# LBANN/DGraph

Measured on AMD Instinct MI355X. Metric: edges_per_s, higher is better.
Workload: dtype fp32

## Files before the change

### csrc/bindings_f32.cpp

```cpp
#include <algorithm>
#include <mutex>
#include <vector>
#include <set>
#include <tuple>
#include <ATen/ATen.h>
#include <c10/core/DeviceGuard.h>
#include <c10/hip/HIPStream.h>
#include <torch/library.h>

#include "check.h"
#include "kernels/kernels.h"

namespace dgraph {
namespace {

hipStream_t stream_of(const at::Tensor& t) {
  return c10::hip::getCurrentHIPStream(t.device().index()).stream();
}

void same_dev(const at::Tensor& t, const at::Tensor& ref, const char* name) {
  TORCH_CHECK(t.is_cuda() && t.device() == ref.device(), "dgraph_amd: ", name,
              " must be a GPU tensor on ", ref.device());
}

// ... 39 lines not shown
              "col must be contiguous int32/int64");
  TORCH_CHECK(x.size(1) == out.size(1), "x/out feature mismatch");
  const at::Tensor* ri = opt(row_ids);
  const at::Tensor* re = opt(rowend);
  const int64_t csr_rows = re ? re->numel() : rowptr.numel() - 1;
  if (re) {
    same_dev(*re, x, "rowend");
    TORCH_CHECK(re->scalar_type() == at::kLong && re->is_contiguous() &&
                    rowptr.numel() >= re->numel(),
                "rowend must be contiguous int64 with at most rowptr's entries");
  }
  const int64_t nrows = ri ? ri->numel() : csr_rows;
  const int64_t* rid = idx64(row_ids, x, nrows, "row_ids");
  const int64_t* rmap = idx64(row_map, x, nrows, "row_map");
  if (!rmap) TORCH_CHECK(out.size(0) >= nrows, "out has fewer rows than the CSR rows");
  auto f32opt = [&](const c10::optional<at::Tensor>& t, const char* name) -> const float* {
    const at::Tensor* p = opt(t);
    if (!p) return nullptr;
    same_dev(*p, x, name);
    TORCH_CHECK(p->scalar_type() == at::kFloat && p->is_contiguous(), name,
                " must be contiguous float32");
    return p->data_ptr<float>();
  };
  SpmmF32Args a;
  a.rowptr = rowptr.data_ptr<int64_t>();
  a.rowend = re ? re->data_ptr<int64_t>() : nullptr;
  a.col = col.data_ptr();
  a.it = col.scalar_type() == at::kInt ? IType::I32 : IType::I64;
  a.ew = f32opt(ew, "edge_weight");
  if (a.ew) TORCH_CHECK(ew->numel() == col.numel(), "edge_weight must be [E]");
  a.col_scale = f32opt(cs, "col_scale");
  a.row_scale = f32opt(rs, "row_scale");
  if (const at::Tensor* p = opt(cmap)) {
    same_dev(*p, x, "col_map");
    TORCH_CHECK(p->scalar_type() == at::kInt && p->is_contiguous(),
                "col_map must be contiguous int32");
    a.col_map = p->data_ptr<int32_t>();
  }
  TORCH_CHECK(spmm_f32_rowgroup_ok(static_cast<int>(x.size(1)), x.stride(0), out.stride(0),
                                   x.data_ptr(), out.data_ptr()),
              "spmm_f32_ex: F % 4 == 0 and 16-B aligned rows/strides required");
  if (const at::Tensor* p = opt(x2)) {
    f32_rows(*p, "x2");
    same_dev(*p, x, "x2");
    TORCH_CHECK(p->size(1) == x.size(1) && p->stride(0) % 4 == 0 &&
                    reinterpret_cast<uintptr_t>(p->data_ptr()) % 16 == 0,
                "x2 must be 16-B aligned, as wide as x, row stride % 4 == 0");
    TORCH_CHECK(nsplit >= 0 && nsplit <= x.size(0) && nsplit < (int64_t(1) << 32),
                "nsplit must be in [0, rows of x]");
    TORCH_CHECK(!a.ew && !a.col_scale,
                "x2 (two sources) is not combined with edge weights / col_scale");
    a.x2 = p->data_ptr<float>();
    a.ldx2 = p->stride(0);
    a.nsplit = nsplit;
  }
  if (const at::Tensor* gt = opt(gate)) {
    f32_rows(*gt, "gate");
    same_dev(*gt, x, "gate");
    TORCH_CHECK(gt->size(1) >= x.size(1) && gt->stride(0) % 4 == 0 &&
                    reinterpret_cast<uintptr_t>(gt->data_ptr()) % 16 == 0,
                "gate must be 16-B aligned with row stride % 4 == 0, width >= F");
    if (!rmap) TORCH_CHECK(gt->size(0) >= nrows, "gate has fewer rows than the output");
    a.gate = gt->data_ptr<float>();
    a.ldgate = gt->stride(0);
  }
  if (const at::Tensor* sa = opt(self_add)) {
    f32_rows(*sa, "self_add");
    same_dev(*sa, x, "self_add");
    const at::Tensor* sm = opt(self_map);
    TORCH_CHECK(sm != nullptr, "self_add needs self_map");
    same_dev(*sm, x, "self_map");
    TORCH_CHECK(sm->scalar_type() == at::kInt && sm->is_contiguous(),
                "self_map must be contiguous int32");
    TORCH_CHECK(sa->size(1) >= x.size(1) && sa->stride(0) % 4 == 0 &&
                    reinterpret_cast<uintptr_t>(sa->data_ptr()) % 16 == 0,
                "self_add must be 16-B aligned with row stride % 4 == 0, width >= F");
    const int64_t max_out = rmap ? out.size(0) : nrows;
    TORCH_CHECK(self_row0 >= 0 && self_row0 + max_out <= sm->numel(),
                "self_map too short for self_row0 + output rows");
    if (sa->size(0) > 0) {
      a.self_add = sa->data_ptr<float>();
      a.self_map = sm->data_ptr<int32_t>();
      a.ld_self = sa->stride(0);
      a.self_row0 = self_row0;
    }
  }
  a.row_ids = rid;
  a.row_map = rmap;
  a.x = x.data_ptr<float>();
  a.ldx = x.stride(0);
  a.out = out.data_ptr<float>();
  a.ldo = out.stride(0);
  a.nrows = nrows;
  a.F = static_cast<int>(x.size(1));
  a.beta = static_cast<float>(beta);
  a.cap = cap;
  a.pass_cols = static_cast<int>(pass_cols);
  if (const at::Tensor* kb = opt(keep_bits)) {
    same_dev(*kb, x, "keep_bits");
    TORCH_CHECK(kb->scalar_type() == at::kInt && kb->dim() == 2 && kb->stride(1) == 1,
                "keep_bits must be int32 [rows, words] with unit column stride");
    TORCH_CHECK(kb->size(1) * 32 >= x.size(1), "keep_bits narrower than the columns");
    TORCH_CHECK(kb->size(0) >= (rmap ? out.size(0) : nrows),
                "keep_bits has fewer rows than the output rows");
    a.keep_bits = reinterpret_cast<const uint32_t*>(kb->data_ptr<int32_t>());
    a.ld_bits = kb->stride(0);
  }
  c10::DeviceGuard g(x.device());
  DG_HIP_CHECK(spmm_f32_run(a, stream_of(x)));
}

void gemm_f32_op(const at::Tensor& A1, const at::Tensor& B1, const c10::optional<at::Tensor>& A2,
                 const c10::optional<at::Tensor>& B2, const c10::optional<at::Tensor>& a_rows,
                 const c10::optional<at::Tensor>& bias, const c10::optional<at::Tensor>& cin,
                 double beta, const c10::optional<at::Tensor>& gate,
                 const c10::optional<at::Tensor>& o_rows, bool relu, const at::Tensor& out,
                 const c10::optional<at::Tensor>& row_scale,
                 const c10::optional<at::Tensor>& send_out,
                 const c10::optional<at::Tensor>& send_ptr,
                 const c10::optional<at::Tensor>& send_pos) {
  f32_rows(A1, "A1");
  f32_rows(B1, "B1");
  f32_rows(out, "out");
  same_dev(B1, A1, "B1");
  same_dev(out, A1, "out");
  const at::Tensor* ar = opt(a_rows);
  const int64_t M = ar ? ar->numel() : A1.size(0);
  const int64_t N = B1.size(1), K1 = A1.size(1);
  TORCH_CHECK(B1.size(0) == K1, "gemm_f32: A1/B1 inner dimension mismatch");
  TORCH_CHECK(out.size(1) == N, "gemm_f32: out width != N");
  TORCH_CHECK(A1.size(0) <= INT32_MAX && M <= INT32_MAX, "gemm_f32: more than 2^31 rows");
  const int64_t* arp = idx64(a_rows, A1, M, "a_rows");
  const int64_t* orp = idx64(o_rows, A1, M, "o_rows");
  if (!orp) TORCH_CHECK(out.size(0) >= M, "gemm_f32: out has fewer than M rows");
  const at::Tensor *a2 = opt(A2), *b2 = opt(B2);
  TORCH_CHECK((a2 == nullptr) == (b2 == nullptr), "gemm_f32: A2 and B2 go together");
  int64_t K2 = 0;
  if (a2) {
    f32_rows(*a2, "A2");
    f32_rows(*b2, "B2");
    same_dev(*a2, A1, "A2");
    same_dev(*b2, A1, "B2");
    K2 = a2->size(1);
    TORCH_CHECK(b2->size(0) == K2 && b2->size(1) == N, "gemm_f32: A2/B2 shape mismatch");
    TORCH_CHECK(a2->size(0) >= M, "gemm_f32: A2 has fewer than M rows");
// ... 191 lines not shown
  DG_HIP_CHECK(apply_keep_bits(g.data_ptr<float>(), g.stride(0),
                               reinterpret_cast<const uint32_t*>(bits.data_ptr<int32_t>()),
                               n, F, stream_of(g), rp));
}

void xent_rows_op(const at::Tensor& z, const at::Tensor& rows, const at::Tensor& y,
                  double scale, const at::Tensor& dz, const at::Tensor& row_loss, int64_t C) {
  f32_rows(z, "z");
  f32_rows(dz, "dz");
  same_dev(rows, z, "rows");
  same_dev(y, z, "y");
  same_dev(dz, z, "dz");
  same_dev(row_loss, z, "row_loss");
  const int64_t n = rows.numel();
  TORCH_CHECK(rows.scalar_type() == at::kLong && rows.is_contiguous() &&
                  y.scalar_type() == at::kLong && y.is_contiguous() && y.numel() == n,
              "rows / y must be contiguous int64 of equal length");
  TORCH_CHECK(C > 0 && C <= 256 && C <= z.size(1) && dz.size(1) >= C && dz.size(1) <= 256 &&
                  dz.size(0) >= n,
              "xent_rows: C <= 256, z and dz at least C wide, dz >= n rows");
  TORCH_CHECK(row_loss.scalar_type() == at::kFloat && row_loss.is_contiguous() &&
                  row_loss.numel() >= n,
              "row_loss must be contiguous float32 with >= n entries");
  c10::DeviceGuard g(z.device());
  DG_HIP_CHECK(xent_rows(z.data_ptr<float>(), z.stride(0), static_cast<int>(C),
                         rows.data_ptr<int64_t>(), y.data_ptr<int64_t>(), n,
                         static_cast<float>(scale), dz.data_ptr<float>(), dz.stride(0),
                         static_cast<int>(dz.size(1)), row_loss.data_ptr<float>(), stream_of(z)));
}

void argmax_hits_op(const at::Tensor& z, const at::Tensor& rows, const at::Tensor& y,
                    const at::Tensor& hit, int64_t C) {
  f32_rows(z, "z");
  same_dev(rows, z, "rows");
  same_dev(y, z, "y");
  same_dev(hit, z, "hit");
  const int64_t n = rows.numel();
  TORCH_CHECK(rows.scalar_type() == at::kLong && rows.is_contiguous() &&
                  y.scalar_type() == at::kLong && y.is_contiguous() && y.numel() == n,
              "rows / y must be contiguous int64 of equal length");
  TORCH_CHECK(hit.scalar_type() == at::kByte && hit.is_contiguous() && hit.numel() >= n,
              "hit must be contiguous uint8 with >= n entries");
  TORCH_CHECK(C > 0 && C <= 256 && C <= z.size(1), "argmax_hits: 0 < C <= 256, C <= width");
  c10::DeviceGuard g(z.device());
  DG_HIP_CHECK(argmax_hits(z.data_ptr<float>(), z.stride(0), static_cast<int>(C),
                           rows.data_ptr<int64_t>(), y.data_ptr<int64_t>(), n,
                           hit.data_ptr<uint8_t>(), stream_of(z)));
}

void set_spmm_f32_config_op(int64_t rowgroup, int64_t pass_cols) {
  set_spmm_f32_config(static_cast<int>(rowgroup), static_cast<int>(pass_cols));
}

void set_f32_sched_op(int64_t spmm_grid, int64_t dynamic, int64_t spmm_xcd) {
  if (spmm_grid >= 0) set_spmm_f32_grid(static_cast<int>(spmm_grid));
  if (spmm_xcd >= 0) set_spmm_f32_xcd(static_cast<int>(spmm_xcd));
  if (dynamic >= 0) set_f32_dynamic(dynamic != 0);
}

void f32_init_op() { DG_HIP_CHECK(work_counters_init()); }

}
}

TORCH_LIBRARY_FRAGMENT(dgraph_amd, m) {
  m.def("set_f32_sched(int spmm_grid=-1, int dynamic=-1, int spmm_xcd=-1) -> ()", &dgraph::set_f32_sched_op);
  m.def("f32_init() -> ()", &dgraph::f32_init_op);
  m.def("set_spmm_f32_config(int rowgroup, int pass_cols=-1) -> ()",
        &dgraph::set_spmm_f32_config_op);
  m.def("spmm_f32_ex(Tensor rowptr, Tensor col, Tensor? edge_weight, Tensor? col_scale, "
        "Tensor? row_scale, Tensor? col_map, Tensor? row_ids, Tensor x, Tensor(a!) out, "
        "float beta=0., int cap=0, Tensor? row_map=None, Tensor? gate=None, "
        "Tensor? self_add=None, Tensor? self_map=None, int self_row0=0, Tensor? rowend=None, "
        "Tensor? x2=None, int nsplit=0, int pass_cols=0, Tensor? keep_bits=None) -> ()");
  m.def("gemm_f32(Tensor A1, Tensor B1, Tensor? A2, Tensor? B2, Tensor? a_rows, Tensor? bias, "
        "Tensor? cin, float beta, Tensor? gate, Tensor? o_rows, bool relu, Tensor(a!) out, "
        "Tensor? row_scale=None, Tensor(b!)? send_out=None, Tensor? send_ptr=None, "
        "Tensor? send_pos=None) -> ()");
  m.def("wgrad_f32(Tensor A1, Tensor? A2, Tensor? a1_rows, Tensor G, Tensor(a!) partials, "
        "int blocks, int fresh_from, Tensor(b!)? col_partials=None) -> ()");
  m.def("wgrad_f32_reduce(Tensor partials, Tensor(a!) out) -> ()");
  m.def("row_keep_bits(Tensor h, Tensor? rows, Tensor(a!) bits) -> ()");
  m.def("apply_keep_bits(Tensor(a!) g, Tensor bits, Tensor? rows=None) -> ()");
  m.def("xent_rows(Tensor z, Tensor rows, Tensor y, float scale, Tensor(a!) dz, "
        "Tensor(b!) row_loss, int C) -> ()");
  m.def("argmax_hits(Tensor z, Tensor rows, Tensor y, Tensor(a!) hit, int C) -> ()");
}

TORCH_LIBRARY_IMPL(dgraph_amd, CUDA, m) {
  m.impl("spmm_f32_ex", &dgraph::spmm_f32_ex_op);
  m.impl("gemm_f32", &dgraph::gemm_f32_op);
  m.impl("wgrad_f32", &dgraph::wgrad_f32_op);
  m.impl("wgrad_f32_reduce", &dgraph::wgrad_f32_reduce_op);
  m.impl("row_keep_bits", &dgraph::row_keep_bits_op);
  m.impl("apply_keep_bits", &dgraph::apply_keep_bits_op);
  m.impl("xent_rows", &dgraph::xent_rows_op);
  m.impl("argmax_hits", &dgraph::argmax_hits_op);
}
```

### csrc/kernels/kernels.h

```cpp
#pragma once
#include <hip/hip_runtime.h>
#include <stdint.h>

#include <initializer_list>

namespace dgraph {

enum class DType : int { F32 = 0, BF16 = 1 };
enum class IType : int { I32 = 0, I64 = 1 };

void set_spmm_config(int variant, int xcd, int pass_cols);

hipError_t spmm_csr(DType dt, IType it, const int64_t* rowptr, const void* col,
                    const float* ew, int heads, int head_dim, const float* col_scale,
                    const float* row_scale, const void* x, int64_t ldx, void* out,
                    int64_t ldo, int64_t nrows, int F, float beta, hipStream_t stream,
                    int64_t cap = 0, const int64_t* row_map = nullptr);

bool spmm_f32_rowgroup_ok(int F, int64_t ldx, int64_t ldo, const void* x, const void* out);
hipError_t spmm_f32_rowgroup(IType it, const int64_t* rowptr, const void* col,
                             const float* ew, const float* col_scale, const float* row_scale,
                             const int32_t* col_map, const int64_t* row_ids, const float* x,
                             int64_t ldx, float* out, int64_t ldo, int64_t nrows, int F,
                             float beta, int64_t cap, const int64_t* row_map,
                             hipStream_t st, const float* gate = nullptr, int64_t ldgate = 0,
                             const float* self_add = nullptr, int64_t ld_self = 0,
                             const int32_t* self_map = nullptr, int64_t self_row0 = 0);
struct SpmmF32Args {
  const int64_t* rowptr = nullptr;
  const int64_t* rowend = nullptr;
  const void* col = nullptr;
  IType it = IType::I32;
  const float* ew = nullptr;
  const float* col_scale = nullptr;
  const float* row_scale = nullptr;
  const int32_t* col_map = nullptr;
  const int64_t* row_ids = nullptr;
  const int64_t* row_map = nullptr;
  const float* x = nullptr;
  int64_t ldx = 0;
  const float* x2 = nullptr;
  int64_t ldx2 = 0;
  int64_t nsplit = 0;
  float* out = nullptr;
  int64_t ldo = 0;
  int64_t nrows = 0;
  int F = 0;
  float beta = 0.f;
  int64_t cap = 0;
  const float* gate = nullptr;
  int64_t ldgate = 0;
  const float* self_add = nullptr;
  int64_t ld_self = 0;
  const int32_t* self_map = nullptr;
  int64_t self_row0 = 0;
  int pass_cols = 0;
  int xcd_remap = 0;
  const uint32_t* keep_bits = nullptr;
  int64_t ld_bits = 0;
  int bits_col0 = 0;
};
hipError_t spmm_f32_run(const SpmmF32Args& a, hipStream_t st);
void set_spmm_f32_pass_cols(int cols);
void set_spmm_f32_config(int rowgroup, int pass_cols);
void set_spmm_f32_grid(int blocks);
void set_spmm_f32_xcd(int on);

hipError_t spmm_hub_partials(DType dt, IType it, const int64_t* seg_beg,
                             const int64_t* seg_end, const void* col, const float* ew,
                             const float* col_scale, const void* x, int64_t ldx,
                             float* partials, int64_t nseg, int F, hipStream_t stream);
hipError_t spmm_hub_reduce(DType dt, const float* partials, const int64_t* hub_seg_ptr,
                           const int64_t* hub_rows, const float* row_scale, void* out,
                           int64_t ldo, int64_t nhub, int F, hipStream_t stream);

hipError_t segment_extreme_fwd(DType dt, IType it, bool minimum, const int64_t* rowptr,
                               const void* col, const void* x, int64_t ldx, void* out,
                               int64_t ldo, int32_t* arg, int64_t lda, int64_t nrows, int F,
                               bool second, const int64_t* row_map, hipStream_t stream);
hipError_t segment_extreme_bwd(DType dt, IType it, const int64_t* t_rowptr, const void* t_col,
                               const int32_t* rel, const void* g, int64_t ldg,
                               const int32_t* arg, int64_t lda, void* out, int64_t ldo,
                               int64_t nrows, int F, bool halo, float beta,
                               hipStream_t stream);

hipError_t segment_pna_fwd(IType it, const int64_t* rowptr, const void* col, const float* x,
                           int64_t ldx, float* mean, int64_t ld_mean, float* sdev,
                           int64_t ld_sdev, float* vmax, int64_t ld_vmax, int32_t* amax,
                           int64_t ld_amax, float* vmin, int64_t ld_vmin, int32_t* amin,
                           int64_t ld_amin, int64_t nrows, int F, float eps, bool second,
                           bool final, const int64_t* prev_rowptr, const int64_t* row_map,
                           hipStream_t stream);
hipError_t segment_pna_bwd(IType it, const int64_t* t_rowptr, const void* t_col,
                           const int32_t* rel, const float* x, int64_t ldx,
                           const float* inv_deg, const float* g_mean, int64_t ld_gmean,
                           const float* g_std, int64_t ld_gstd, const float* mean,
                           int64_t ld_mean, const float* sdev, int64_t ld_sdev,
                           const float* g_max, int64_t ld_gmax, const int32_t* amax,
                           int64_t ld_amax, const float* g_min, int64_t ld_gmin,
                           const int32_t* amin, int64_t ld_amin, float* out, int64_t ldo,
                           int64_t nrows, int F, bool halo, float beta, hipStream_t stream);

int64_t segment_softmax_dt_parts(int64_t nrows);
hipError_t segment_softmax_fwd(IType it, const int64_t* rowptr, const void* col, const float* x,
                               int64_t ldx, const float* t, float* out, int64_t ldo, float* lse,
                               int64_t ldl, int64_t nrows, int F, bool second,
                               const int64_t* row_map, hipStream_t stream);
hipError_t segment_softmax_bwd(IType it, const int64_t* t_rowptr, const void* t_col,
                               const float* x, int64_t ldx, const float* t, const float* g,
                               int64_t ldg, const float* out_fwd, int64_t ldof,
                               const float* lse, int64_t ldl, float* dx, int64_t lddx,
                               float* dt_part, int64_t nrows, int F, hipStream_t stream);

int64_t segment_softmax_edge_dt_parts(int64_t nrows);
hipError_t segment_softmax_edge_fwd(IType it, const int64_t* rowptr, const void* col,
                                    const float* x, int64_t ldx, const float* e, int64_t lde,
                                    const float* t, float* out, int64_t ldo, float* lse,
                                    int64_t ldl, int64_t nrows, int F, bool relu, float eps,
                                    bool second, const int64_t* row_map, hipStream_t stream);
// ... 268 lines not shown
```

### csrc/kernels/spmm_f32.hip

```cpp
#include "../common.h"
#include "kernels.h"

namespace dgraph {
namespace {

typedef float f32x2 __attribute__((ext_vector_type(2)));

template <typename IdxT, int LPR, int WMODE, bool CMAP, bool TWO, bool KB = false,
          bool GS = false>
__global__ __launch_bounds__(256) void spmm_f32_rowgroup_kernel(SpmmF32Args a) {
  constexpr int VEC = 4;
  constexpr int G = kWave / LPR;
  constexpr int U = LPR < 8 ? LPR : 8;
  constexpr bool HAS_EW = (WMODE & 1) != 0;
  constexpr bool HAS_CS = (WMODE & 2) != 0;
  const IdxT* __restrict__ col = static_cast<const IdxT*>(a.col);
  const int64_t* __restrict__ rowptr = a.rowptr;
  const int lane = threadIdx.x & (kWave - 1);
  const int g = lane / LPR;
  const int l = lane % LPR;
  const int wv = threadIdx.x >> 6;
  __shared__ uint8_t inv[CMAP ? 4 * 64 : 1];
  const int64_t nrows = a.nrows;
  const int F = a.F;
  const int64_t ngroups = (nrows + G - 1) / G;
  int64_t blk = blockIdx.x;
  if (a.xcd_remap) {
    const int64_t full = static_cast<int64_t>(gridDim.x) & ~int64_t(7);
    if (blk < full) blk = (blk & 7) * (full >> 3) + (blk >> 3);
  }
  const int64_t q0 = (blk * blockDim.x + threadIdx.x) >> 6;
  const int64_t qstep = (static_cast<int64_t>(gridDim.x) * blockDim.x) >> 6;
  const int f = l * VEC;
  const bool active = f < F;
  const float* xf = a.x + (active ? f : 0);
  const float* x2f = TWO ? a.x2 + (active ? f : 0) : nullptr;
  const uint64_t ldx = static_cast<uint64_t>(a.ldx);
  const uint64_t ldx2 = static_cast<uint64_t>(a.ldx2);
  const uint32_t ns = static_cast<uint32_t>(a.nsplit);
  const int cap = a.cap;
  auto row_ptr = [&](uint32_t c) -> const float* {
    if constexpr (TWO) {
      return c < ns ? xf + static_cast<uint64_t>(c) * ldx
                    : x2f + static_cast<uint64_t>(c - ns) * ldx2;
    } else {
      return xf + static_cast<uint64_t>(c) * ldx;
    }
  };
  for (int64_t q = q0; q < ngroups; q += qstep) {
    const int64_t r = q * G + g;
    const bool has_row = r < nrows;
    const int64_t rr = has_row ? (a.row_ids ? a.row_ids[r] : r) : 0;
    const int64_t s = has_row ? rowptr[rr] : 0;
    const int64_t deg1 = has_row ? (a.rowend ? a.rowend[rr] : rowptr[rr + 1]) - s : 0;
    const int deg = static_cast<int>(deg1 > cap ? cap : deg1);
    int32_t m_top = -1;
    if constexpr (GS) m_top = a.self_map[a.self_row0 + (has_row ? r : 0)];
    int maxdeg = deg;
#pragma unroll
    for (int off = LPR; off < kWave; off <<= 1) {
      const int o = __shfl_xor(maxdeg, off, kWave);
      maxdeg = o > maxdeg ? o : maxdeg;
    }
    f32x2 acc[VEC / 2];
#pragma unroll
    for (int i = 0; i < VEC / 2; ++i) acc[i] = f32x2{0.f, 0.f};
    auto load_c = [&](int k) -> int64_t {
      const IdxT c = col[k < deg ? s + k : 0];
      return k < deg ? static_cast<int64_t>(c) : int64_t(0);
    };
    auto load_w = [&](int64_t& c, int k) -> float {
      float w = k < deg ? 1.f : 0.f;
      if constexpr (CMAP) {
        const int32_t m = a.col_map[c];
        w = m >= 0 ? w : 0.f;
        c = m >= 0 ? m : 0;
      }
      if constexpr (HAS_EW) w *= a.ew[k < deg ? s + k : 0];
      if constexpr (HAS_CS) w *= a.col_scale[c];
      return w;
    };
    int64_t my_c = 0;
    float my_w = 0.f;
    if (maxdeg > 0) {
      my_c = load_c(l);
      my_w = load_w(my_c, l);
    }
    for (int k0 = 0; k0 < maxdeg; k0 += LPR) {
      const int kn = k0 + LPR + l;
// ... 19 lines not shown
#pragma unroll
          for (int u = 0; u < U; ++u) {
            const int j = j0 + u;
            const int src = j < cnt ? static_cast<int>(inv[wv * kWave + g * LPR + j]) : 0;
            c[u] = static_cast<uint32_t>(__shfl(static_cast<int>(my_c), g * LPR + src, kWave));
            const float ww = __shfl(my_w, g * LPR + src, kWave);
            w[u] = j < cnt ? ww : 0.f;
          }
#pragma unroll
          for (int u = 0; u < U; ++u) v[u] = *reinterpret_cast<const uint4*>(row_ptr(c[u]));
#pragma unroll
          for (int u = 0; u < U; ++u) {
            const f32x2 ww{w[u], w[u]};
            const f32x2 t0{__uint_as_float(v[u].x), __uint_as_float(v[u].y)};
            const f32x2 t1{__uint_as_float(v[u].z), __uint_as_float(v[u].w)};
            acc[0] = __builtin_elementwise_fma(t0, ww, acc[0]);
            acc[1] = __builtin_elementwise_fma(t1, ww, acc[1]);
          }
        }
        my_w = load_w(nx_c, kn);
        my_c = nx_c;
        continue;
      }
#pragma unroll
      for (int j0 = 0; j0 < LPR; j0 += U) {
        if (j0 > 0 && k0 + j0 >= maxdeg) break;
        uint4 v[U];
        uint32_t c[U];
        float w[U];
#pragma unroll
        for (int u = 0; u < U; ++u)
          c[u] = static_cast<uint32_t>(
              __shfl(static_cast<int>(my_c), g * LPR + j0 + u, kWave));
        if (j0 == 0) nx_c = load_c(kn);
#pragma unroll
        for (int u = 0; u < U; ++u) v[u] = *reinterpret_cast<const uint4*>(row_ptr(c[u]));
#pragma unroll
        for (int u = 0; u < U; ++u) w[u] = __shfl(my_w, g * LPR + j0 + u, kWave);
#pragma unroll
        for (int u = 0; u < U; ++u) {
          const f32x2 ww{w[u], w[u]};
          const f32x2 t0{__uint_as_float(v[u].x), __uint_as_float(v[u].y)};
          const f32x2 t1{__uint_as_float(v[u].z), __uint_as_float(v[u].w)};
          acc[0] = __builtin_elementwise_fma(t0, ww, acc[0]);
          acc[1] = __builtin_elementwise_fma(t1, ww, acc[1]);
        }
      }
      my_w = load_w(nx_c, kn);
      my_c = nx_c;
    }
    if (has_row && active) {
      const int64_t orow = (!GS && a.row_map) ? a.row_map[r] : r;
      const float rs = a.row_scale ? a.row_scale[orow] : 1.f;
      float* o = a.out + orow * a.ldo + f;
      const float beta = a.beta;
      float4 res;
      if (beta != 0.f) {
        const float4 old = *reinterpret_cast<const float4*>(o);
        res.x = fmaf(acc[0].x, rs, beta * old.x);
        res.y = fmaf(acc[0].y, rs, beta * old.y);
        res.z = fmaf(acc[1].x, rs, beta * old.z);
        res.w = fmaf(acc[1].y, rs, beta * old.w);
      } else {
        res.x = acc[0].x * rs;
        res.y = acc[0].y * rs;
        res.z = acc[1].x * rs;
        res.w = acc[1].y * rs;
      }
      if constexpr (GS) {
        const float4 sv = *reinterpret_cast<const float4*>(
            a.self_add + static_cast<int64_t>(m_top >= 0 ? m_top : 0) * a.ld_self + f);
        const float4 gv = *reinterpret_cast<const float4*>(a.gate + orow * a.ldgate + f);
        res.x = m_top >= 0 ? res.x + sv.x : res.x;
        res.y = m_top >= 0 ? res.y + sv.y : res.y;
        res.z = m_top >= 0 ? res.z + sv.z : res.z;
        res.w = m_top >= 0 ? res.w + sv.w : res.w;
        res.x = gv.x > 0.f ? res.x : 0.f;
        res.y = gv.y > 0.f ? res.y : 0.f;
        res.z = gv.z > 0.f ? res.z : 0.f;
        res.w = gv.w > 0.f ? res.w : 0.f;
      } else if (a.self_add) {
        const int32_t m = a.self_map[a.self_row0 + orow];
        if (m >= 0) {
          const float4 sv = *reinterpret_cast<const float4*>(a.self_add + m * a.ld_self + f);
          res.x += sv.x;
          res.y += sv.y;
          res.z += sv.z;
          res.w += sv.w;
        }
      }
      if (!GS && a.gate) {
        const float4 gv = *reinterpret_cast<const float4*>(a.gate + orow * a.ldgate + f);
        res.x = gv.x > 0.f ? res.x : 0.f;
        res.y = gv.y > 0.f ? res.y : 0.f;
        res.z = gv.z > 0.f ? res.z : 0.f;
        res.w = gv.w > 0.f ? res.w : 0.f;
      }
      if constexpr (KB) {
        const int c = a.bits_col0 + f;
        const uint32_t w = a.keep_bits[orow * a.ld_bits + (c >> 5)] >> (c & 31);
        res.x = (w & 1u) ? res.x : 0.f;
        res.y = (w & 2u) ? res.y : 0.f;
        res.z = (w & 4u) ? res.z : 0.f;
        res.w = (w & 8u) ? res.w : 0.f;
      }
      *reinterpret_cast<float4*>(o) = res;
    }
  }
}

int g_f32_grid_cap = 0;
int g_f32_xcd = 0;

template <typename IdxT>
hipError_t launch_f32_rg(const SpmmF32Args& a, hipStream_t st) {
  const int lanes = (a.F + 3) / 4;
  const int LPR = lanes <= 8 ? 8 : lanes <= 16 ? 16 : lanes <= 32 ? 32 : 64;
  const int64_t G = kWave / LPR;
  const int64_t ngroups = (a.nrows + G - 1) / G;
  int64_t blocks = (ngroups + 3) / 4;
  SpmmF32Args ka = a;
  ka.xcd_remap = g_f32_xcd ? 1 : 0;
  if (g_f32_grid_cap > 0 && blocks > g_f32_grid_cap) {
    blocks = g_f32_grid_cap;
    ka.xcd_remap = 0;
  }
  if (blocks > 0x7fffffff) return hipErrorInvalidValue;
  const int wmode = (a.ew != nullptr ? 1 : 0) | (a.col_scale != nullptr ? 2 : 0);
  const bool cmap = a.col_map != nullptr;
  const bool two = a.x2 != nullptr;
  const bool kb = a.keep_bits != nullptr;
  if (two && wmode != 0) return hipErrorInvalidValue;
  if (kb && (two || cmap || wmode != 0)) return hipErrorInvalidValue;
  if (kb) {
#define DG_F32_KB(LPR_)                                                                      \
    if (LPR == LPR_) {                                                                       \
      hipLaunchKernelGGL((spmm_f32_rowgroup_kernel<IdxT, LPR_, 0, false, false, true>), grid, \
                         block, 0, st, ka);                                                  \
      return hipGetLastError();                                                              \
    }
    dim3 grid(static_cast<unsigned>(blocks)), block(256);
    DG_F32_KB(8) DG_F32_KB(16) DG_F32_KB(32) DG_F32_KB(64)
#undef DG_F32_KB
    return hipErrorInvalidValue;
  }
  dim3 grid(static_cast<unsigned>(blocks)), block(256);
  if (cmap && wmode == 0 && a.gate && a.self_add && a.self_map && !a.row_map) {
#define DG_F32_GS(LPR_, T_)                                                                    \
    if (LPR == LPR_ && two == T_) {                                                            \
      hipLaunchKernelGGL((spmm_f32_rowgroup_kernel<IdxT, LPR_, 0, true, T_, false, true>), grid, \
                         block, 0, st, ka);                                                    \
      return hipGetLastError();                                                                \
    }
    DG_F32_GS(8, false) DG_F32_GS(16, false) DG_F32_GS(32, false) DG_F32_GS(64, false)
    DG_F32_GS(8, true) DG_F32_GS(16, true) DG_F32_GS(32, true) DG_F32_GS(64, true)
#undef DG_F32_GS
  }
#define DG_F32_K(LPR_, W_, C_, T_)                                                         \
  if (LPR == LPR_ && wmode == W_ && cmap == C_ && two == T_) {                              \
    hipLaunchKernelGGL((spmm_f32_rowgroup_kernel<IdxT, LPR_, W_, C_, T_>), grid, block, 0, \
                       st, ka);                                                             \
    return hipGetLastError();                                                               \
  }
#define DG_F32(LPR_)                                                                        \
  DG_F32_K(LPR_, 0, false, false) DG_F32_K(LPR_, 1, false, false)                           \
  DG_F32_K(LPR_, 2, false, false) DG_F32_K(LPR_, 3, false, false)                           \
  DG_F32_K(LPR_, 0, true, false) DG_F32_K(LPR_, 1, true, false)                             \
  DG_F32_K(LPR_, 2, true, false) DG_F32_K(LPR_, 3, true, false)                             \
  DG_F32_K(LPR_, 0, false, true) DG_F32_K(LPR_, 0, true, true)
  DG_F32(8)
  DG_F32(16)
  DG_F32(32)
  DG_F32(64)
#undef DG_F32_K
#undef DG_F32
  return hipErrorInvalidValue;
}

int g_f32_pass_cols = 64;

}

void set_spmm_f32_pass_cols(int cols) { g_f32_pass_cols = cols > 0 ? cols : 64; }

void set_spmm_f32_grid(int blocks) { g_f32_grid_cap = blocks > 0 ? blocks : 0; }

void set_spmm_f32_xcd(int on) { g_f32_xcd = on ? 1 : 0; }

bool spmm_f32_rowgroup_ok(int F, int64_t ldx, int64_t ldo, const void* x, const void* out) {
  auto al = [](const void* p) { return (reinterpret_cast<uintptr_t>(p) % 16) == 0; };
  return F % 4 == 0 && ldx % 4 == 0 && ldo % 4 == 0 && al(x) && al(out) &&
         ldx < (int64_t(1) << 40);
}

hipError_t spmm_f32_run(const SpmmF32Args& args, hipStream_t st) {
  if (args.nrows <= 0 || args.F <= 0) return hipSuccess;
  auto al = [](const void* p) { return (reinterpret_cast<uintptr_t>(p) & 15) == 0; };
  if (args.self_add && (!args.self_map || !al(args.self_add) || args.ld_self % 4))
    return hipErrorInvalidValue;
  if (args.gate && (!al(args.gate) || args.ldgate % 4)) return hipErrorInvalidValue;
  if (!spmm_f32_rowgroup_ok(args.F, args.ldx, args.ldo, args.x, args.out))
    return hipErrorInvalidValue;
  if (args.x2 && (!al(args.x2) || args.ldx2 % 4 || args.nsplit < 0 ||
                  args.nsplit >= (int64_t(1) << 32)))
    return hipErrorInvalidValue;
  SpmmF32Args a = args;
  a.cap = (args.cap > 0 && args.cap < (int64_t(1) << 30)) ? args.cap : (1 << 30);
  int pc = args.pass_cols > 0 ? args.pass_cols : g_f32_pass_cols;
  pc = pc > 256 ? 256 : (pc < 16 ? 16 : pc - pc % 4);
  for (int c0 = 0; c0 < args.F; c0 += pc) {
    SpmmF32Args p = a;
    p.F = args.F - c0 < pc ? args.F - c0 : pc;
    p.x = args.x + c0;
    p.x2 = args.x2 ? args.x2 + c0 : nullptr;
    p.out = args.out + c0;
    p.gate = args.gate ? args.gate + c0 : nullptr;
    p.self_add = args.self_add ? args.self_add + c0 : nullptr;
    p.bits_col0 = args.bits_col0 + c0;
    const hipError_t err = args.it == IType::I32 ? launch_f32_rg<int32_t>(p, st)
                                                 : launch_f32_rg<int64_t>(p, st);
    if (err != hipSuccess) return err;
  }
  return hipSuccess;
}

hipError_t spmm_f32_rowgroup(IType it, const int64_t* rowptr, const void* col,
                             const float* ew, const float* col_scale, const float* row_scale,
                             const int32_t* col_map, const int64_t* row_ids, const float* x,
                             int64_t ldx, float* out, int64_t ldo, int64_t nrows, int F,
                             float beta, int64_t cap, const int64_t* row_map,
                             hipStream_t st, const float* gate, int64_t ldgate,
                             const float* self_add, int64_t ld_self, const int32_t* self_map,
                             int64_t self_row0) {
  SpmmF32Args a{};
  a.rowptr = rowptr;
  a.col = col;
  a.it = it;
  a.ew = ew;
  a.col_scale = col_scale;
  a.row_scale = row_scale;
  a.col_map = col_map;
  a.row_ids = row_ids;
  a.row_map = row_map;
  a.x = x;
  a.ldx = ldx;
  a.out = out;
  a.ldo = ldo;
  a.nrows = nrows;
  a.F = F;
  a.beta = beta;
  a.cap = cap;
  a.gate = gate;
  a.ldgate = ldgate;
  a.self_add = self_add;
  a.ld_self = ld_self;
  a.self_map = self_map;
  a.self_row0 = self_row0;
  return spmm_f32_run(a, st);
}

}
```

### dgraph_amd/models/sage_fused.py

```python
from __future__ import annotations

import os
from typing import List, Optional, Tuple

import torch

from ..comm.alltoallv import AllToAllV
from ..ops import f32 as F32
from ..ops import kernels as K
from ..parallel.dist_graph import DistGraph
from ..parallel.reorder import graph_locality
from ..utils.config import ExecutorConfig

PLAN_LINK_GBPS = 153.0
PLAN_SPMM_TBPS = 13.0
PLAN_GEMM_TFPS = 120.0
PLAN_HBM_TBPS = 5.0


def _ranges(a: int, b: int, step: int) -> List[Tuple[int, int]]:
    return [(r, min(b, r + step)) for r in range(a, b, step)]


def _pad_to(n: int, m: int) -> int:
# ... 105 lines not shown
        return self.nnz_int + self.nnz_halo

    def halo_degree(self) -> torch.Tensor:
        if self.mid is None:
            return torch.zeros(self.rp.numel() - 1, dtype=torch.long, device=self.rp.device)
        return self.rp[1:] - self.mid

    def rows(self, r0: int, r1: int, part: str):
        if self.mid is None or part == "all":
            if part == "halo":
                raise ValueError("no halo entries")
            return self.rp[r0:r1 + 1], None
        if part == "int":
            return self.rp[r0:r1], self.mid[r0:r1]
        return self.mid[r0:r1], self.rp[r0 + 1:r1 + 1]

    def memory_bytes(self) -> int:
        if self.mid is None:
            return 0
        return self.rp.numel() * 8 + self.mid.numel() * 8 + self.col.numel() * 4


class _Budget:

    def __init__(self, free: int, need_h: int, other: int, margin: int, wA: int, wB: int):
        self.free, self.need_h, self.other, self.margin = free, need_h, other, margin
        self.wA, self.wB = wA, wB
        self.sub_bytes = 0
        self.decisions: list = []

    def note(self, what: str, nbytes: int, taken: bool) -> None:
        self.decisions.append({"what": what, "gb": round(nbytes / 2**30, 2),
                               "room_gb": round(self.room() / 2**30, 2), "taken": bool(taken)})

    def room(self) -> int:
        return self.free - self.need_h - self.other

    def describe(self, halo_bytes: int, dev) -> str:
        return (f"FusedSAGE: activations {self.need_h / 2**30:.1f} GiB (halo rows "
                f"{halo_bytes / 2**30:.1f}) + workspace {self.other / 2**30:.1f} GiB exceed the "
                f"{self.free / 2**30:.1f} GiB free on {dev}")


class FusedSAGE:

    def __init__(self, model, graph: DistGraph, x: torch.Tensor, train_idx: torch.Tensor,
                 y_train: torch.Tensor, eval_idx: torch.Tensor, y_eval: torch.Tensor,
                 eval_is_val: torch.Tensor, n_train: int, chunk_rows: int = 0,
                 release_graph: bool = False, reserve_bytes: int = 0,
                 config: Optional[ExecutorConfig] = None):
        if not supported(model, x):
            raise ValueError("FusedSAGE: unsupported model/feature shape")
        self.cfg = config if config is not None else ExecutorConfig.from_env()
        dev = x.device
        self.dev = dev
        if dev.type == "cuda":
            from .. import _native

            with torch.cuda.device(dev):
                _native.ops().f32_init()
            if os.environ.get("DGRAPH_F32_DYNAMIC") is not None:
                _native.ops().set_f32_sched(-1, int(os.environ["DGRAPH_F32_DYNAMIC"]))
        self.d0_in = x.shape[1]
        self.d0 = _in_width(self.d0_in, len(model.layers))
        if self.d0 != self.d0_in:
            xp = torch.zeros(x.shape[0], self.d0, dtype=x.dtype, device=dev)
            xp[:, :self.d0_in] = x
            x = xp
        self.model, self.g, self.x = model, graph, x.contiguous()
        self.L, self.H = graph.L, graph.H
        self.nl = len(model.layers)
        self.hid = model.layers[0].out_dim
        self.C = model.layers[-1].out_dim
        self.Cp = _width_at_least(self.C, (64, 128, 176, 192, 256))
        self.Cg = _width_at_least(_pad_to(self.C, 32) if self.C > 128 else self.C,
                                  (128, 176, 192, 256))
        self.inv_n = 1.0 / max(int(n_train), 1)
        self._setup_rows(graph, train_idx, y_train, eval_idx, y_eval, eval_is_val)
        self._setup_adjacency(graph, release_graph)
        b = self._plan_memory(graph, reserve_bytes)
        self._plan_chunks(chunk_rows, b)
        self._allocate(graph, b)
        self.row_loss = torch.zeros(self.T.numel(), dtype=torch.float32, device=dev)
        self.hit = torch.zeros(self.E.numel(), dtype=torch.uint8, device=dev)
        self.E_val_l = self.E_val.long()
        self.correct = torch.zeros(2, dtype=torch.long, device=dev)
        self.record = False
        self._events: list = []
        self._packs: dict = {}
        self._agg0_in_h = False
        self._tune_passes()

    def _setup_rows(self, graph: DistGraph, train_idx, y_train, eval_idx, y_eval,
                    eval_is_val) -> None:
        dev, L = self.dev, self.L
        t, tp = torch.sort(train_idx.long())
        self.T, self.yT = t.contiguous(), y_train[tp].contiguous()
        e, ep = torch.sort(eval_idx.long())
        self.E, self.yE = e.contiguous(), y_eval[ep].contiguous()
        self.E_val = eval_is_val[ep].contiguous()
        self.inv_deg = graph.inv_deg
        self.invdegT = self.inv_deg[self.T].contiguous()
        it_t, _, sub = graph._restricted(self.T)
        parts = [self.T, it_t.compact_rows().row_map.long()]
        if sub is not None:
            parts.append(sub[4].long())
# ... 808 lines not shown

    def step(self) -> torch.Tensor:
        g, x = self.g, self.x
        nl, hid, C, Cp, Cg = self.nl, self.hid, self.C, self.Cp, self.Cg
        P = self._params()
        dev = self.dev
        self._events = []
        self._mark("fwd_l0")
        nnz = self.nnz_it + self.nnz_h
        hin, hin_halo = x, (g._static_halo(x) if g.send_map is not None else None)
        halos = []
        reuse0, self._agg0_in_h = self._agg0_in_h, False
        for l in range(nl - 1):
            ws, wn, b = P[l]
            if l == 0:
                ws, wn = self._pad_in(ws), self._pad_in(wn)
            else:
                ws, wn = ws.detach().contiguous(), wn.detach().contiguous()
            hout = self.h[l]
            bias = b.detach()

            keep_s = self.aS_keep if l == nl - 2 else None

            sends = not self.stream and not (self.pf is not None and l == nl - 2)

            def consume(ci, a, hin=hin, hout=hout, ws=ws, wn=wn, bias=bias, keep_s=keep_s,
                        sends=sends):
                r0, r1 = self.chunks[ci]
                if keep_s is not None:
                    self._keep_s_rows(ci, a, keep_s)
                self._gemm(hin[r0:r1], ws, a, wn, bias=bias, relu=True, out=hout[r0:r1],
                           send=self._send_arg(r0, r1, hout.shape[1]) if sends else None)

            if self.stream and l > 0 and not self.cfg.stream_fill:
                self._stream_fwd(hin, hout, f"fwd_l{l}")
                for ci, (r0, r1) in enumerate(self.chunks):
                    if r1 > r0:
                        consume(ci, hout[r0:r1])
                halos.append(None)
            elif self.stream and l > 0:
                agg = self.agg_full[:, :hin.shape[1]]
                self._stream_fwd(hin, agg, f"fwd_l{l}",
                                 fill=lambda hin=hin, ws=ws, bias=bias, hout=hout:
                                 self._gemm(hin, ws, bias=bias, out=hout))
                for ci, (r0, r1) in enumerate(self.chunks):
                    if r1 > r0:
                        a = agg[r0:r1]
                        if keep_s is not None:
                            self._keep_s_rows(ci, a, keep_s)
                        self._gemm(a, wn, cin=hout[r0:r1], beta=1.0, relu=True,
                                   out=hout[r0:r1])
                halos.append(None)
            elif l == 0 and reuse0:
                for ci, (r0, r1) in enumerate(self.chunks):
                    if r1 > r0:
                        consume(ci, hout[r0:r1, :self.d0])
                halos.append(hin_halo)
            else:
                store = hout[self.Li:] if (l > 0 and hin.shape[1] == hout.shape[1] and
                                           self.use_store["hidden"]) else None
                keep = self.agg0 if l == 0 else None
                halos.append(self._layer(hin, hin_halo, consume, hin.shape[1], f"fwd_l{l}",
                                         store=store, keep=keep))
            if not (l == 0 and reuse0):
                self.edges_aggregated += nnz
            hin = hout
            hin_halo = None if (self.stream or (self.pf is not None and l == nl - 2)) \
                else self._exchange(hout, l)
            self._mark(f"fwd_l{l + 1}" if l + 1 < nl - 1 else "fwd_out")
        ws, wn, b = P[nl - 1]
        wsp = torch.zeros(hid, Cp, device=dev)
        wsp[:, :C] = ws.detach()
        wnp = torch.zeros(hid, Cp, device=dev)
        wnp[:, :C] = wn.detach()
        bp = torch.zeros(Cp, device=dev)
        bp[:C] = b.detach()
        self.acc_out_s.reset()
        self.acc_out_n.reset()
        hl = hin
        if self.pf is not None:
            Pb, Li = self.pf, self.Li
            tw = self._aggT_issue(hl)
            self._gemm(hl[Li:], wnp, out=Pb[Li:],
                       send=None if self.stream else self._send_arg(Li, self.L, Cp))
            out_pf = lambda ci, a: self._out_chunk(ci, a, hl, wsp, wnp, bp, pf=True)
            if self.stream:
                self._stream_fwd(Pb, self.agg_full[:, :Cp], "fwd_out",
                                 fill=(lambda: self._gemm(hl[:Li], wnp, out=Pb[:Li]))
                                 if Li > 0 else None)
                for ci, (r0, r1) in enumerate(self.chunks):
                    if r1 > r0:
                        out_pf(ci, self.agg_full[r0:r1, :Cp])
                hl_halo = None
            else:
                pend = self._exchange_pf(Pb)
                if Li > 0:
                    self._gemm(hl[:Li], wnp, out=Pb[:Li])
                hl_halo = self._layer(Pb, pend, out_pf, Cp, "fwd_out",
                                      store=self.agg_full if self.use_store["out"] else None)
            self._aggT_finish(hl, tw)
        elif self.stream:
            zs = self.zself
            self._stream_fwd(hl, self.agg_full, "fwd_out",
                             fill=None if zs is None else
                             (lambda: self._gemm(hl, wsp, bias=bp, out=zs)))
            for ci, (r0, r1) in enumerate(self.chunks):
                if r1 > r0:
                    self._out_chunk(ci, self.agg_full[r0:r1, :hid], hl, wsp, wnp, bp)
            hl_halo = None
# ... 251 lines not shown
```

Baseline: 5.677 billion.

## Merge column passes of f32 SpMM into one launch; single GEMM for layer 0

When the feature width exceeds the pass width, the f32 SpMM now launches every column pass as one grid and derives the pass from the block index. Previously it issued one launch per column slice. The merged path is taken only when inputs and output do not overlap in memory and no grid cap is set, so the passes can safely run concurrently. Layer 0 with reused aggregation now runs one full-height GEMM instead of one per chunk when there are no send plans or keep masks. This cuts launch overhead and tail effects, but running all passes at once changes cache reuse and the order of the work.

```diff
diff --git a/csrc/bindings_f32.cpp b/csrc/bindings_f32.cpp
--- a/csrc/bindings_f32.cpp
+++ b/csrc/bindings_f32.cpp
@@ -115,6 +115,7 @@
                 "x2 (two sources) is not combined with edge weights / col_scale");
     a.x2 = p->data_ptr<float>();
     a.ldx2 = p->stride(0);
+    a.x2_rows = p->size(0);
     a.nsplit = nsplit;
   }
   if (const at::Tensor* gt = opt(gate)) {
@@ -145,6 +146,7 @@
       a.self_add = sa->data_ptr<float>();
       a.self_map = sm->data_ptr<int32_t>();
       a.ld_self = sa->stride(0);
+      a.self_rows = sa->size(0);
       a.self_row0 = self_row0;
     }
   }
@@ -154,6 +156,8 @@
   a.ldx = x.stride(0);
   a.out = out.data_ptr<float>();
   a.ldo = out.stride(0);
+  a.x_rows = x.size(0);
+  a.out_rows = out.size(0);
   a.nrows = nrows;
   a.F = static_cast<int>(x.size(1));
   a.beta = static_cast<float>(beta);
@@ -451,9 +455,11 @@
   set_spmm_f32_config(static_cast<int>(rowgroup), static_cast<int>(pass_cols));
 }
 
-void set_f32_sched_op(int64_t spmm_grid, int64_t dynamic, int64_t spmm_xcd) {
+void set_f32_sched_op(int64_t spmm_grid, int64_t dynamic, int64_t spmm_xcd,
+                      int64_t spmm_merge) {
   if (spmm_grid >= 0) set_spmm_f32_grid(static_cast<int>(spmm_grid));
   if (spmm_xcd >= 0) set_spmm_f32_xcd(static_cast<int>(spmm_xcd));
+  if (spmm_merge >= 0) set_spmm_f32_merge(static_cast<int>(spmm_merge));
   if (dynamic >= 0) set_f32_dynamic(dynamic != 0);
 }
 
@@ -463,7 +469,8 @@
 }
 
 TORCH_LIBRARY_FRAGMENT(dgraph_amd, m) {
-  m.def("set_f32_sched(int spmm_grid=-1, int dynamic=-1, int spmm_xcd=-1) -> ()", &dgraph::set_f32_sched_op);
+  m.def("set_f32_sched(int spmm_grid=-1, int dynamic=-1, int spmm_xcd=-1, int spmm_merge=-1) -> ()",
+        &dgraph::set_f32_sched_op);
   m.def("f32_init() -> ()", &dgraph::f32_init_op);
   m.def("set_spmm_f32_config(int rowgroup, int pass_cols=-1) -> ()",
         &dgraph::set_spmm_f32_config_op);
diff --git a/csrc/kernels/kernels.h b/csrc/kernels/kernels.h
--- a/csrc/kernels/kernels.h
+++ b/csrc/kernels/kernels.h
@@ -59,12 +59,17 @@
   const uint32_t* keep_bits = nullptr;
   int64_t ld_bits = 0;
   int bits_col0 = 0;
+  int64_t x_rows = 0, x2_rows = 0, out_rows = 0, self_rows = 0;
+  int npass = 1;
+  int F_total = 0;
+  uint32_t blocks_per_pass = 0;
 };
 hipError_t spmm_f32_run(const SpmmF32Args& a, hipStream_t st);
 void set_spmm_f32_pass_cols(int cols);
 void set_spmm_f32_config(int rowgroup, int pass_cols);
 void set_spmm_f32_grid(int blocks);
 void set_spmm_f32_xcd(int on);
+void set_spmm_f32_merge(int on);
 
 hipError_t spmm_hub_partials(DType dt, IType it, const int64_t* seg_beg,
                              const int64_t* seg_end, const void* col, const float* ew,
diff --git a/csrc/kernels/spmm_f32.hip b/csrc/kernels/spmm_f32.hip
--- a/csrc/kernels/spmm_f32.hip
+++ b/csrc/kernels/spmm_f32.hip
@@ -22,19 +22,22 @@
   const int wv = threadIdx.x >> 6;
   __shared__ uint8_t inv[CMAP ? 4 * 64 : 1];
   const int64_t nrows = a.nrows;
-  const int F = a.F;
+  const uint32_t bpp = a.blocks_per_pass;
+  const uint32_t pass = blockIdx.x / bpp;
+  const int c0 = static_cast<int>(pass) * a.pass_cols;
+  const int F = a.F_total - c0 < a.F ? a.F_total - c0 : a.F;
   const int64_t ngroups = (nrows + G - 1) / G;
-  int64_t blk = blockIdx.x;
+  int64_t blk = blockIdx.x - pass * bpp;
   if (a.xcd_remap) {
-    const int64_t full = static_cast<int64_t>(gridDim.x) & ~int64_t(7);
+    const int64_t full = static_cast<int64_t>(bpp) & ~int64_t(7);
     if (blk < full) blk = (blk & 7) * (full >> 3) + (blk >> 3);
   }
   const int64_t q0 = (blk * blockDim.x + threadIdx.x) >> 6;
-  const int64_t qstep = (static_cast<int64_t>(gridDim.x) * blockDim.x) >> 6;
+  const int64_t qstep = (static_cast<int64_t>(bpp) * blockDim.x) >> 6;
   const int f = l * VEC;
   const bool active = f < F;
-  const float* xf = a.x + (active ? f : 0);
-  const float* x2f = TWO ? a.x2 + (active ? f : 0) : nullptr;
+  const float* xf = a.x + c0 + (active ? f : 0);
+  const float* x2f = TWO ? a.x2 + c0 + (active ? f : 0) : nullptr;
   const uint64_t ldx = static_cast<uint64_t>(a.ldx);
   const uint64_t ldx2 = static_cast<uint64_t>(a.ldx2);
   const uint32_t ns = static_cast<uint32_t>(a.nsplit);
@@ -160,7 +163,7 @@
     if (has_row && active) {
       const int64_t orow = (!GS && a.row_map) ? a.row_map[r] : r;
       const float rs = a.row_scale ? a.row_scale[orow] : 1.f;
-      float* o = a.out + orow * a.ldo + f;
+      float* o = a.out + c0 + orow * a.ldo + f;
       const float beta = a.beta;
       float4 res;
       if (beta != 0.f) {
@@ -177,8 +180,9 @@
       }
       if constexpr (GS) {
         const float4 sv = *reinterpret_cast<const float4*>(
-            a.self_add + static_cast<int64_t>(m_top >= 0 ? m_top : 0) * a.ld_self + f);
-        const float4 gv = *reinterpret_cast<const float4*>(a.gate + orow * a.ldgate + f);
+            a.self_add + c0 + static_cast<int64_t>(m_top >= 0 ? m_top : 0) * a.ld_self + f);
+        const float4 gv =
+            *reinterpret_cast<const float4*>(a.gate + c0 + orow * a.ldgate + f);
         res.x = m_top >= 0 ? res.x + sv.x : res.x;
         res.y = m_top >= 0 ? res.y + sv.y : res.y;
         res.z = m_top >= 0 ? res.z + sv.z : res.z;
@@ -190,7 +194,8 @@
       } else if (a.self_add) {
         const int32_t m = a.self_map[a.self_row0 + orow];
         if (m >= 0) {
-          const float4 sv = *reinterpret_cast<const float4*>(a.self_add + m * a.ld_self + f);
+          const float4 sv =
+              *reinterpret_cast<const float4*>(a.self_add + c0 + m * a.ld_self + f);
           res.x += sv.x;
           res.y += sv.y;
           res.z += sv.z;
@@ -198,14 +203,15 @@
         }
       }
       if (!GS && a.gate) {
-        const float4 gv = *reinterpret_cast<const float4*>(a.gate + orow * a.ldgate + f);
+        const float4 gv =
+            *reinterpret_cast<const float4*>(a.gate + c0 + orow * a.ldgate + f);
         res.x = gv.x > 0.f ? res.x : 0.f;
         res.y = gv.y > 0.f ? res.y : 0.f;
         res.z = gv.z > 0.f ? res.z : 0.f;
         res.w = gv.w > 0.f ? res.w : 0.f;
       }
       if constexpr (KB) {
-        const int c = a.bits_col0 + f;
+        const int c = a.bits_col0 + c0 + f;
         const uint32_t w = a.keep_bits[orow * a.ld_bits + (c >> 5)] >> (c & 31);
         res.x = (w & 1u) ? res.x : 0.f;
         res.y = (w & 2u) ? res.y : 0.f;
@@ -219,21 +225,33 @@
 
 int g_f32_grid_cap = 0;
 int g_f32_xcd = 0;
+int g_f32_merge = 1;
+
+int f32_lpr(int width) {
+  const int lanes = (width + 3) / 4;
+  return lanes <= 8 ? 8 : lanes <= 16 ? 16 : lanes <= 32 ? 32 : 64;
+}
+
+int64_t f32_pass_blocks(int64_t nrows, int width) {
+  const int64_t G = kWave / f32_lpr(width);
+  const int64_t ngroups = (nrows + G - 1) / G;
+  return (ngroups + 3) / 4;
+}
 
 template <typename IdxT>
 hipError_t launch_f32_rg(const SpmmF32Args& a, hipStream_t st) {
-  const int lanes = (a.F + 3) / 4;
-  const int LPR = lanes <= 8 ? 8 : lanes <= 16 ? 16 : lanes <= 32 ? 32 : 64;
-  const int64_t G = kWave / LPR;
-  const int64_t ngroups = (a.nrows + G - 1) / G;
-  int64_t blocks = (ngroups + 3) / 4;
+  const int LPR = f32_lpr(a.F);
+  int64_t blocks = f32_pass_blocks(a.nrows, a.F);
   SpmmF32Args ka = a;
   ka.xcd_remap = g_f32_xcd ? 1 : 0;
   if (g_f32_grid_cap > 0 && blocks > g_f32_grid_cap) {
+    if (a.npass != 1) return hipErrorInvalidValue;
     blocks = g_f32_grid_cap;
     ka.xcd_remap = 0;
   }
-  if (blocks > 0x7fffffff) return hipErrorInvalidValue;
+  if (blocks <= 0 || a.npass < 1 || blocks * a.npass > 0x7fffffff) return hipErrorInvalidValue;
+  ka.blocks_per_pass = static_cast<uint32_t>(blocks);
+  blocks *= a.npass;
   const int wmode = (a.ew != nullptr ? 1 : 0) | (a.col_scale != nullptr ? 2 : 0);
   const bool cmap = a.col_map != nullptr;
   const bool two = a.x2 != nullptr;
@@ -294,6 +312,8 @@
 void set_spmm_f32_grid(int blocks) { g_f32_grid_cap = blocks > 0 ? blocks : 0; }
 
 void set_spmm_f32_xcd(int on) { g_f32_xcd = on ? 1 : 0; }
+
+void set_spmm_f32_merge(int on) { g_f32_merge = on ? 1 : 0; }
 
 bool spmm_f32_rowgroup_ok(int F, int64_t ldx, int64_t ldo, const void* x, const void* out) {
   auto al = [](const void* p) { return (reinterpret_cast<uintptr_t>(p) % 16) == 0; };
@@ -316,9 +336,30 @@
   a.cap = (args.cap > 0 && args.cap < (int64_t(1) << 30)) ? args.cap : (1 << 30);
   int pc = args.pass_cols > 0 ? args.pass_cols : g_f32_pass_cols;
   pc = pc > 256 ? 256 : (pc < 16 ? 16 : pc - pc % 4);
+  a.pass_cols = pc;
+  const int npass = (args.F + pc - 1) / pc;
+  auto apart = [&](const float* p, int64_t rows, int64_t ld) {
+    if (!p) return true;
+    if (rows <= 0 || args.out_rows <= 0) return false;
+    const float* pe = p + (rows - 1) * ld + args.F;
+    const float* oe = args.out + (args.out_rows - 1) * args.ldo + args.F;
+    return pe <= args.out || oe <= p;
+  };
+  if (g_f32_merge && npass > 1 && g_f32_grid_cap == 0 &&
+      f32_pass_blocks(args.nrows, pc) * npass <= 0x7fffffff &&
+      apart(args.x, args.x_rows, args.ldx) && apart(args.x2, args.x2_rows, args.ldx2) &&
+      apart(args.self_add, args.self_rows, args.ld_self)) {
+    a.F = pc;
+    a.F_total = args.F;
+    a.npass = npass;
+    return args.it == IType::I32 ? launch_f32_rg<int32_t>(a, st)
+                                 : launch_f32_rg<int64_t>(a, st);
+  }
+  a.npass = 1;
   for (int c0 = 0; c0 < args.F; c0 += pc) {
     SpmmF32Args p = a;
     p.F = args.F - c0 < pc ? args.F - c0 : pc;
+    p.F_total = p.F;
     p.x = args.x + c0;
     p.x2 = args.x2 ? args.x2 + c0 : nullptr;
     p.out = args.out + c0;
diff --git a/dgraph_amd/models/sage_fused.py b/dgraph_amd/models/sage_fused.py
--- a/dgraph_amd/models/sage_fused.py
+++ b/dgraph_amd/models/sage_fused.py
@@ -181,6 +181,7 @@
         if not supported(model, x):
             raise ValueError("FusedSAGE: unsupported model/feature shape")
         self.cfg = config if config is not None else ExecutorConfig.from_env()
+        self.l0_one_gemm = True
         dev = x.device
         self.dev = dev
         if dev.type == "cuda":
@@ -1095,9 +1096,14 @@
                                    out=hout[r0:r1])
                 halos.append(None)
             elif l == 0 and reuse0:
-                for ci, (r0, r1) in enumerate(self.chunks):
-                    if r1 > r0:
-                        consume(ci, hout[r0:r1, :self.d0])
+                if self.l0_one_gemm and (not sends or self.send_plan is None) \
+                        and keep_s is None and self.L > 0:
+                    self._gemm(hin[:self.L], ws, hout[:self.L, :self.d0], wn, bias=bias,
+                               relu=True, out=hout[:self.L])
+                else:
+                    for ci, (r0, r1) in enumerate(self.chunks):
+                        if r1 > r0:
+                            consume(ci, hout[r0:r1, :self.d0])
                 halos.append(hin_halo)
             else:
                 store = hout[self.Li:] if (l > 0 and hin.shape[1] == hout.shape[1] and
```

Result: no change. 5.721 billion (median of 6 runs) (+0.8%).
